# vicpc00/td-vc-gan

Measured on AMD Instinct MI355X. Metric: audio-seconds/sec (G+D train step, stage-1), higher is better.
Workload: dtype f32 (fp32 storage and accumulation everywhere; FiLM cond_var.2 forward and weight-grad as split-bf16 x6 products -- three exact bf16 pieces per operand, six piece products on the bf16 MFMA, fp32 accumulate: fp32-level accuracy; every other kernel exact-fp32 MFMA)

## Files before the change

td-vc-gan_amd/csrc/conv_api.hip:

```cpp
#include "../../include/tdvc.h"
#include "launch.h"
#include "conv_lean.h"
#include "conv_small_group.h"
#include "api_util.h"

using namespace tdvc;

static inline bool al16(const void* p) { return (((uintptr_t)p) & 15) == 0; }
static inline bool ok_bs(const void* p, long bs) { return !p || (bs < (1L << 31)); }
static inline bool vec_ptr(const void* p, long bs) { return !p || (al16(p) && (bs & 3) == 0); }
static inline float scale_or_1(float s) { return s == 0.f ? 1.f : s; }

static int lean_xfk(const tdvc_xform& x, float* slope, float* scale, const float** aux, long* aux_bs) {
  *scale = scale_or_1(x.scale); *aux = x.aux; *aux_bs = x.aux_bs; *slope = x.slope;
  switch (x.kind) {
    case TDVC_XF_NONE: *slope = 1.f; *aux = nullptr; return LXF_ACT;
    case TDVC_XF_LRELU: *aux = nullptr; return (x.slope >= 0.f && x.slope <= 1.f) ? LXF_ACT : -1;
    case TDVC_XF_FILM_LRELU: return (x.slope >= 0.f && x.slope <= 1.f) ? LXF_FILM : -1;
    case TDVC_XF_MASK_LRELU: return LXF_MASK_LRELU;
    case TDVC_XF_MASK_TANH: return LXF_MASK_TANH;
    default: return -1;
  }
}

namespace tdvc { int g_force_generic = 0; }
extern "C" void tdvc_set_force_generic(int on) { g_force_generic = on; }

static Xf to_xf(const tdvc_xform& x) {
  Xf r; r.kind = x.kind; r.slope = x.slope; r.scale = scale_or_1(x.scale);
  r.aux = x.aux; r.aux_bs = x.aux_bs; return r;
}

static int check_desc(const tdvc_conv_desc* d) {
  if (!d) return tdvc_fail(TDVC_EINVAL, "null desc");
  if (d->B <= 0 || d->Cin <= 0 || d->Cout <= 0 || d->Tin <= 0 || d->Tout <= 0 || d->K <= 0 || d->stride <= 0 ||
      d->dilation <= 0 || d->groups <= 0 || d->pad < 0)
    return tdvc_fail(TDVC_EINVAL, "conv desc: non-positive dimension");
  if (d->Cin % d->groups || d->Cout % d->groups) return tdvc_fail(TDVC_EINVAL, "conv desc: channels not divisible by groups");
  if (d->stride > 1 && d->dilation != 1) return tdvc_fail(TDVC_EUNSUPPORTED, "strided conv with dilation");
  if (d->reflect && (d->stride != 1 || d->kind != TDVC_CONV)) return tdvc_fail(TDVC_EUNSUPPORTED, "reflect padding needs stride 1 conv");
  if (d->reflect && d->pad >= d->Tin) return tdvc_fail(TDVC_EINVAL, "reflect padding must be smaller than the input length");
  if (d->w_cin < 0 || d->w_cin_off < 0) return tdvc_fail(TDVC_EINVAL, "conv desc: negative weight channel window");
  if (d->w_cin > 0) {
    if (d->groups != 1 || d->kind != TDVC_CONV) return tdvc_fail(TDVC_EUNSUPPORTED, "weight channel window needs a plain conv with groups == 1");
    if (d->w_cin_off + d->Cin > d->w_cin) return tdvc_fail(TDVC_EINVAL, "conv desc: weight channel window out of range");
  }
  if (d->kind == TDVC_CONV) {
    long expect = ((long)d->Tin + 2L * d->pad - (long)d->dilation * (d->K - 1) - 1) / d->stride + 1;
    if (expect != d->Tout) return tdvc_fail(TDVC_EINVAL, "conv desc: Tout does not match conv arithmetic");
  } else if (d->kind == TDVC_CONV_TRANSPOSE) {
    if (d->stride < 2) return tdvc_fail(TDVC_EUNSUPPORTED, "transposed conv needs stride >= 2");
    long expect = ((long)d->Tin - 1) * d->stride - 2L * d->pad + (d->K - 1) + 1;
    if (d->Tout > expect + d->stride - 1 || d->Tout < expect) return tdvc_fail(TDVC_EINVAL, "conv desc: Tout does not match transposed conv arithmetic");
  } else return tdvc_fail(TDVC_EINVAL, "conv desc: unknown kind");
  return TDVC_OK;
}

static inline int ceil_div(int a, int b) { return (a + b - 1) / b; }

enum { TRY_NEXT = 1 };
static int launch_rc(hipError_t e, bool may_decline = false) {
  if (e == hipSuccess) return TDVC_OK;
  if (may_decline && e == hipErrorNotSupported) return TRY_NEXT;
  return tdvc_fail(TDVC_ELAUNCH, hipGetErrorString(e));
}

template <class P>
static void set_reduced(P& p, int mode, int R, int C, int T, const tdvc_conv_desc* d) {
  const int s = d->stride;
  p.mode = mode; p.R = R; p.Cred = C; p.N = T; p.J = ceil_div(d->K, s); p.d = 1;
  if (mode == MODE_DIRECT) p.d = d->dilation;
  else if (mode == MODE_DOWN) p.Cred = C * s;
  else { p.R = R * s; p.N = (T - 1 + d->pad) / s + 1; }
}

static bool small_group_ok(const tdvc_conv_desc* d) {
  return !g_force_generic && g_knob[2] == 0 && d->kind == TDVC_CONV && d->groups >= 16 && d->Cin == 4 * d->groups && d->Cout == 4 * d->groups &&
         d->dilation == 1 && !d->reflect && d->w_cin == 0 && d->stride >= 2 && d->stride <= 8 && d->K <= 48;
}
static void small_group_base(const tdvc_conv_desc* d, SmallGroupP& q) {
  q.B = d->B; q.G = d->groups; q.Tin = d->Tin; q.Tout = d->Tout; q.K = d->K; q.s = d->stride; q.pad = d->pad;
  q.in_scale = 1.f; q.out_scale = 1.f; q.dy_scale = 1.f;
}

static bool use_mfma(const GemmConvP& p) {
  if (g_force_generic) return false;
  if (p.R <= 2 && p.x.Cg == 1 && p.Cy_g <= 2) return false;
  return (long)p.Cred * p.J >= 7;
}

template <int MODE>
static int run_gemm(GemmConvP& p, int B, hipStream_t st) {
  return launch_rc(use_mfma(p) ? launch_conv_gemm<MODE>(p, B, st) : launch_conv_scalar<MODE>(p, B, st));
}

static int dispatch_gemm(GemmConvP& p, int B, hipStream_t st) {
  switch (p.mode) {
    case MODE_DIRECT: return run_gemm<MODE_DIRECT>(p, B, st);
    case MODE_DOWN: return run_gemm<MODE_DOWN>(p, B, st);
    default: return run_gemm<MODE_UP>(p, B, st);
  }
}

enum { CV_SMALL_GROUP, CV_LEAN, CV_GENERIC };

static bool lean_shape_ok(const tdvc_conv_desc* d) {
  return !g_force_generic && d->kind == TDVC_CONV && d->stride == 1 && d->groups == 1 && d->Tin == d->Tout && ((d->Tin & 3) == 0 || d->Tin <= 80);
}

static bool lean_fill(const tdvc_conv_desc* d, const tdvc_xform& xf, const long (&bs)[7], LeanP& q, int* xfk) {
  long aux_bs;
  *xfk = lean_xfk(xf, &q.slope, &q.in_scale, &q.aux, &aux_bs);
  const struct { const void* p; long bs; int* q_bs; } opnds[] = {{q.x, bs[0], &q.x_bs}, {q.y, bs[1], &q.y_bs}, {q.res, bs[2], &q.res_bs}, {q.add, bs[3], &q.add_bs},
      {q.mx, bs[4], &q.mx_bs}, {q.gb, bs[5], &q.gb_bs}, {q.dgb, bs[6], &q.dgb_bs}, {q.aux, aux_bs, &q.aux_bs}};
  bool ok = *xfk >= 0 && (q.Cw & 3) == 0 && al16(q.w), vec = (d->Tin & 3) == 0;
  for (const auto& o : opnds) { ok = ok && ok_bs(o.p, o.bs); vec = vec && vec_ptr(o.p, o.bs); *o.q_bs = (int)o.bs; }
  q.T = d->Tin; q.K = d->K; q.d = d->dilation; q.vec = vec ? 1 : 0;
  return ok && (vec || d->Tin <= 80);
}

static int fwd_route(const tdvc_conv_desc* d, const tdvc_conv_fwd_args* a, int from, LeanP& q, int* xfk) {
  if (from <= CV_SMALL_GROUP && small_group_ok(d) && a->x_xf.kind <= TDVC_XF_LRELU && !a->res && !a->add && !a->bias3) return CV_SMALL_GROUP;
  if (from <= CV_LEAN && lean_shape_ok(d) && (d->Cin & 3) == 0) {
    q.x = a->x; q.y = a->y; q.bias = a->bias; q.bias3 = a->bias3; q.res = a->res; q.add = a->add;
    q.w = a->w + (long)d->w_cin_off * d->K; q.Cw = (d->w_cin > 0 ? d->w_cin : d->Cin) * d->K;
    q.Cin = d->Cin; q.Cout = d->Cout; q.pad = d->pad; q.reflect = d->reflect;
    q.post = a->post_act; q.out_scale = scale_or_1(a->out_scale); q.add_scale = 1.f; q.m_slope = a->post_slope;
    q.sbits = a->sign_bits; q.sb_bs = (int)a->sign_bits_bs;
    if (lean_fill(d, a->x_xf, {a->x_bs, a->y_bs, a->res_bs, a->add_bs, 0, 0, 0}, q, xfk)) return CV_LEAN;
  }
  return CV_GENERIC;
}

extern "C" int tdvc_conv_fwd(const tdvc_conv_desc* d, const tdvc_conv_fwd_args* a, void* stream) {
  if (int rc = check_desc(d)) return rc;
  if (!a || !a->x || !a->w || !a->y) return tdvc_fail(TDVC_EINVAL, "conv_fwd: null pointer");
  hipStream_t st = (hipStream_t)stream;
  LeanP q = {};
  int xfk = 0, route = CV_SMALL_GROUP;
  while ((route = fwd_route(d, a, route, q, &xfk)) != CV_GENERIC) {
    hipError_t e;
    if (route == CV_SMALL_GROUP) {
      SmallGroupP g = {};
      small_group_base(d, g);
      g.x = a->x; g.x_bs = a->x_bs; g.w = a->w; g.bias = a->bias; g.y = a->y; g.y_bs = a->y_bs;
      g.act_in = a->x_xf.kind == TDVC_XF_LRELU; g.slope_in = a->x_xf.slope; g.in_scale = scale_or_1(a->x_xf.scale);
      g.post = a->post_act; g.post_slope = a->post_slope; g.out_scale = scale_or_1(a->out_scale);
      e = launch_small_group_fwd(g, st);
    } else e = launch_conv_lean(q, d->B, xfk, EPI_FWD, st);
    const int rc = launch_rc(e, true);
    if (rc != TRY_NEXT) return rc;
    ++route;
  }
  if (a->sign_bits) return tdvc_fail(TDVC_EUNSUPPORTED, "conv_fwd: sign_bits needs a stride-1 conv with Tout % 32 == 0, Tout > 80 and 16-byte aligned operands");
  const int Cin_g = d->Cin / d->groups, Cout_g = d->Cout / d->groups;
  GemmConvP p = {};
  p.x.p = a->x; p.x.bs = a->x_bs; p.x.T = d->Tin; p.x.Cg = Cin_g; p.x.xf = to_xf(a->x_xf);
  p.w = a->w; p.K = d->K; p.s = d->stride; p.pad = d->pad; p.groups = d->groups;
  p.y = a->y; p.y_bs = a->y_bs; p.Ty = d->Tout; p.Cy_g = Cout_g;
  p.epi = EPI_FWD; p.bias = a->bias; p.bias3 = a->bias3; p.res = a->res; p.res_bs = a->res_bs;
  p.post = a->post_act; p.post_slope = a->post_slope; p.out_scale = scale_or_1(a->out_scale);
  p.add = a->add; p.add_bs = a->add_bs; p.add_scale = 1.f;
  p.w_sg = (long)Cout_g * Cin_g * d->K;
  if (d->kind == TDVC_CONV) {
    p.w_sm = (long)Cin_g * d->K; p.w_sc = d->K;
    if (d->w_cin > 0) { p.w_sm = (long)d->w_cin * d->K; p.w += (long)d->w_cin_off * d->K; }
    set_reduced(p, d->stride == 1 ? MODE_DIRECT : MODE_DOWN, Cout_g, Cin_g, d->Tout, d);
    p.reflect = d->reflect;
  } else {
    p.w_sm = d->K; p.w_sc = (long)Cout_g * d->K;
    set_reduced(p, MODE_UP, Cout_g, Cin_g, d->Tout, d);
  }
  return dispatch_gemm(p, d->B, st);
}

static int dgrad_route(const tdvc_conv_desc* d, const tdvc_conv_dgrad_args* a, int from, LeanP& q, int* xfk) {
  if (from <= CV_SMALL_GROUP && small_group_ok(d) && a->epilogue == TDVC_DG_PLAIN && !a->add &&
      (a->dy_xf.kind == TDVC_XF_NONE || (a->dy_xf.kind == TDVC_XF_MASK_LRELU && a->dy_xf.aux))) return CV_SMALL_GROUP;
  if (from <= CV_LEAN && a->wt && lean_shape_ok(d) && (d->Cout & 3) == 0 && (d->K - 1) * d->dilation - d->pad >= 0) {
    q.x = a->dy; q.y = a->dx; q.add = a->add; q.mx = a->x_in; q.gb = a->gb; q.dgb = a->dgb;
    q.Cw = d->Cout * d->K; q.w = a->wt + (long)d->w_cin_off * q.Cw;
    q.Cin = d->Cout; q.Cout = d->Cin; q.pad = (d->K - 1) * d->dilation - d->pad; q.flip = 1; q.mirror = d->reflect ? d->pad : 0;
    q.out_scale = 1.f; q.add_scale = a->add_scale; q.m_slope = a->slope;
    if (a->epilogue == TDVC_DG_MASK_LRELU && a->x_sign_bits) { q.mbits = a->x_sign_bits; q.mb_bs = (int)a->x_sign_bits_bs; }
    if (lean_fill(d, a->dy_xf, {a->dy_bs, a->dx_bs, 0, a->add_bs, a->x_in_bs, a->gb_bs, a->dgb_bs}, q, xfk)) return CV_LEAN;
  }
  return CV_GENERIC;
}

extern "C" int tdvc_conv_dgrad(const tdvc_conv_desc* d, const tdvc_conv_dgrad_args* a, void* stream) {
  if (int rc = check_desc(d)) return rc;
  if (!a || !a->dy || !a->w || !a->dx) return tdvc_fail(TDVC_EINVAL, "conv_dgrad: null pointer");
  if (a->epilogue < TDVC_DG_PLAIN || a->epilogue > TDVC_DG_FILM) return tdvc_fail(TDVC_EINVAL, "conv_dgrad: unknown epilogue");
  const int epi = a->epilogue == TDVC_DG_PLAIN ? EPI_PLAIN : (a->epilogue == TDVC_DG_MASK_LRELU ? EPI_MASK : EPI_FILM);
  if (epi == EPI_MASK && !a->x_in && !a->x_sign_bits) return tdvc_fail(TDVC_EINVAL, "conv_dgrad: mask epilogue needs x_in");
  if (epi == EPI_FILM && (!a->x_in || !a->gb || !a->dgb)) return tdvc_fail(TDVC_EINVAL, "conv_dgrad: FiLM epilogue needs x_in, gb, dgb");
  hipStream_t st = (hipStream_t)stream;
  LeanP q = {};
  int xfk = 0, route = CV_SMALL_GROUP;
  while ((route = dgrad_route(d, a, route, q, &xfk)) != CV_GENERIC) {
    hipError_t e;
    if (route == CV_SMALL_GROUP) {
      SmallGroupP g = {};
      small_group_base(d, g);
      g.dy = a->dy; g.dy_bs = a->dy_bs; g.w = a->w; g.y = a->dx; g.y_bs = a->dx_bs;
      g.dy_scale = scale_or_1(a->dy_xf.scale);
      if (a->dy_xf.kind == TDVC_XF_MASK_LRELU) { g.mask = a->dy_xf.aux; g.mask_bs = a->dy_xf.aux_bs; g.m_slope = a->dy_xf.slope; }
      e = launch_small_group_dgrad(g, st);
    } else {
      e = launch_conv_lean(q, d->B, xfk, epi, st);
      if (e == hipErrorNotSupported && q.mbits && a->x_in) {
        q.mbits = nullptr;
        e = launch_conv_lean(q, d->B, xfk, epi, st);
      }
    }
    const int rc = launch_rc(e, true);
    if (rc != TRY_NEXT) return rc;
    ++route;
  }
  if (epi == EPI_MASK && !a->x_in)
    return tdvc_fail(TDVC_EUNSUPPORTED, "conv_dgrad: x_sign_bits without x_in needs a stride-1 conv with Tin % 32 == 0, Tin > 80 and 16-byte aligned operands");
  const int Cin_g = d->Cin / d->groups, Cout_g = d->Cout / d->groups;
  GemmConvP p = {};
  p.x.p = a->dy; p.x.bs = a->dy_bs; p.x.T = d->Tout; p.x.Cg = Cout_g; p.x.xf = to_xf(a->dy_xf);
  p.w = a->w; p.K = d->K; p.s = d->stride; p.pad = d->pad; p.groups = d->groups;
  p.y = a->dx; p.y_bs = a->dx_bs; p.Ty = d->Tin; p.Cy_g = Cin_g;
  p.add = a->add; p.add_bs = a->add_bs; p.add_scale = a->add_scale;
  p.w_sg = (long)Cout_g * Cin_g * d->K;
  p.epi = epi;
  if (epi != EPI_PLAIN) { p.mx = a->x_in; p.mx_bs = a->x_in_bs; p.m_slope = a->slope; }
  if (epi == EPI_FILM) { p.gb = a->gb; p.gb_bs = a->gb_bs; p.dgb = a->dgb; p.dgb_bs = a->dgb_bs; }
  if (d->kind == TDVC_CONV) {
    p.w_sm = d->K; p.w_sc = (long)Cin_g * d->K;
    if (d->w_cin > 0) { p.w_sc = (long)d->w_cin * d->K; p.w += (long)d->w_cin_off * d->K; }
    set_reduced(p, d->stride == 1 ? MODE_DIRECT : MODE_UP, Cin_g, Cout_g, d->Tin, d);
    if (d->stride == 1) {
      p.tap_flip = 1; p.pad = (d->K - 1) * d->dilation - d->pad;
      if (p.pad < 0) return tdvc_fail(TDVC_EUNSUPPORTED, "conv_dgrad: padding larger than the receptive field");
      p.mirror_pad = d->reflect ? d->pad : 0;
    }
  } else {
    p.w_sm = (long)Cout_g * d->K; p.w_sc = d->K;
    set_reduced(p, MODE_DOWN, Cin_g, Cout_g, d->Tin, d);
  }
  return dispatch_gemm(p, d->B, st);
}

static void fill_wgrad(const tdvc_conv_desc* d, const tdvc_conv_wgrad_args* a, WgradP& p) {
  const int Cin_g = d->Cin / d->groups, Cout_g = d->Cout / d->groups;
  p.groups = d->groups; p.K = d->K; p.s = d->stride; p.pad = d->pad;
  p.w_sg = (long)Cout_g * Cin_g * d->K; p.w_sc = d->K;
  if (d->kind == TDVC_CONV) {
    if (a) { p.a.p = a->dy; p.a.bs = a->dy_bs; p.a.xf = to_xf(a->dy_xf); p.x.p = a->x; p.x.bs = a->x_bs; p.x.xf = to_xf(a->x_xf); }
    p.a.T = d->Tout; p.a.Cg = Cout_g; p.x.T = d->Tin; p.x.Cg = Cin_g;
    p.w_sm = (long)Cin_g * d->K;
    set_reduced(p, d->stride == 1 ? MODE_DIRECT : MODE_DOWN, Cout_g, Cin_g, d->Tout, d);
    p.reflect = d->reflect;
  } else {
    if (a) { p.a.p = a->x; p.a.bs = a->x_bs; p.a.xf = to_xf(a->x_xf); p.x.p = a->dy; p.x.bs = a->dy_bs; p.x.xf = to_xf(a->dy_xf); }
    p.a.T = d->Tin; p.a.Cg = Cin_g; p.x.T = d->Tout; p.x.Cg = Cout_g;
    p.w_sm = (long)Cout_g * d->K;
    set_reduced(p, MODE_DOWN, Cin_g, Cout_g, d->Tin, d);
  }
}

static bool wgrad_use_mfma(const WgradP& p) {
  if (g_force_generic) return false;
  if (p.R <= 2 && p.x.Cg == 1) return false;
  if (!wgrad_mfma_supported(p.J)) return false;
  return true;
}

static bool wgrad_lean_ok(const tdvc_conv_desc* d) {
  const bool wide = d->Cout >= 32 && d->Cin >= 32;
  return !g_force_generic && d->kind == TDVC_CONV && d->stride == 1 && d->groups == 1 && d->Tin == d->Tout &&
         (d->Tout > 128 || wide) && wgrad_lean_supported(d->Cout, d->Cin, d->K, d->dilation);
}

static bool wgrad_x6_desc_ok(const tdvc_conv_desc* d) {
  return wgrad_lean_ok(d) && d->w_cin == 0 && wgrad_x6_ok(d->Cout, d->Cin, d->Tout, d->K, d->dilation, d->pad, d->reflect);
}

enum { WG_SMALL_GROUP, WG_X6, WG_LEAN, WG_MFMA, WG_SCALAR };
struct WgPlan {
  int route;
  int nslab; long sstride;
  bool bias;
  int bpb;
  size_t bytes;
};

static WgPlan wgrad_plan(const tdvc_conv_desc* d, const tdvc_conv_wgrad_args* a, WgradP& p, int from) {
  const long wsize = (long)d->groups * p.w_sg;
  WgPlan pl = {};
  auto slabs = [&](int route, int nslab, bool bias) {
    pl.route = route; pl.nslab = nslab; pl.bias = bias; pl.sstride = wsize + (bias ? d->Cout : 0);
    pl.bytes = (size_t)nslab * (size_t)pl.sstride * sizeof(float);
    return pl;
  };
  if (from <= WG_SMALL_GROUP && small_group_ok(d) &&
      (!a || (a->x_xf.kind <= TDVC_XF_LRELU && (a->dy_xf.kind == TDVC_XF_NONE || (a->dy_xf.kind == TDVC_XF_MASK_LRELU && a->dy_xf.aux))))) {
    pl.route = WG_SMALL_GROUP; pl.bias = true; pl.bytes = small_group_wgrad_workspace(d->B, d->groups, d->K);
    return pl;
  }
  if (from <= WG_X6 && wgrad_x6_desc_ok(d) &&
      (!a || (a->x_xf.kind <= TDVC_XF_LRELU && a->dy_xf.kind == TDVC_XF_NONE && scale_or_1(a->x_xf.scale) == 1.f && scale_or_1(a->dy_xf.scale) == 1.f &&
              (a->x_xf.kind == TDVC_XF_NONE || (a->x_xf.slope > 0.f && a->x_xf.slope <= 1.f)) &&
              al16(a->x) && al16(a->dy) && (a->x_bs & 3) == 0 && (a->dy_bs & 3) == 0))) {
    int nt, tpb, nslab;
    wgrad_x6_plan(d->Cout, d->Tout, d->B, &nt, &tpb, &nslab);
    return slabs(WG_X6, nslab, true);
  }
  if (from <= WG_LEAN && wgrad_lean_ok(d)) return slabs(WG_LEAN, wgrad_lean_nslab(d->Cout, d->Cin, d->Tout, d->K, d->B), true);
  if (from <= WG_MFMA && wgrad_use_mfma(p)) {
    const int nslab = wgrad_geometry(p, d->B, &pl.bpb);
    return slabs(WG_MFMA, nslab, false);
  }
  pl.route = WG_SCALAR;
  return pl;
}

extern "C" size_t tdvc_conv_wgrad_workspace(const tdvc_conv_desc* d) {
  if (check_desc(d)) return 0;
  WgradP p = {};
  fill_wgrad(d, nullptr, p);
  size_t need = 0;
  for (int from = WG_SMALL_GROUP; from <= WG_LEAN; ) {
    const WgPlan pl = wgrad_plan(d, nullptr, p, from);
    if (pl.bytes > need) need = pl.bytes;
    from = pl.route + 1;
  }
  return need;
}

extern "C" int tdvc_conv_wgrad(const tdvc_conv_desc* d, const tdvc_conv_wgrad_args* a, void* stream) {
  if (int rc = check_desc(d)) return rc;
  if (!a || !a->x || !a->dy) return tdvc_fail(TDVC_EINVAL, "conv_wgrad: null pointer");
  hipStream_t st = (hipStream_t)stream;
  WgradP p = {};
  fill_wgrad(d, a, p);
  const long wsize = (long)d->groups * p.w_sg;
  float* dw = (a->dw && d->w_cin > 0) ? a->dw + (long)d->w_cin_off * d->K : a->dw;
  const long dw_rs = d->w_cin > 0 ? (long)d->w_cin * d->K : p.w_sm;
  bool bias_done = false;
  for (int from = WG_SMALL_GROUP; a->dw; ) {
    const WgPlan pl = wgrad_plan(d, a, p, from);
    if (pl.route != WG_SMALL_GROUP && pl.bytes && (!a->workspace || a->workspace_bytes < pl.bytes))
      return tdvc_fail(TDVC_EWORKSPACE, "conv_wgrad: workspace too small");
    hipError_t e;
    if (pl.route == WG_SMALL_GROUP) {
      SmallGroupP q = {};
      small_group_base(d, q);
      q.x = a->x; q.x_bs = a->x_bs; q.dy = a->dy; q.dy_bs = a->dy_bs;
      q.act_in = a->x_xf.kind == TDVC_XF_LRELU; q.slope_in = a->x_xf.slope; q.in_scale = scale_or_1(a->x_xf.scale);
      q.dy_scale = scale_or_1(a->dy_xf.scale);
      if (a->dy_xf.kind == TDVC_XF_MASK_LRELU) { q.mask = a->dy_xf.aux; q.mask_bs = a->dy_xf.aux_bs; q.m_slope = a->dy_xf.slope; }
      e = launch_small_group_wgrad(q, a->dw, a->dbias, a->workspace, a->workspace_bytes, st);
    } else if (pl.route == WG_X6 || pl.route == WG_LEAN) {
      WgLeanP q = {};
      q.a = p.a; q.x = p.x; q.R = d->Cout; q.Cin = d->Cin; q.N = d->Tout; q.pad = d->pad; q.K = d->K; q.reflect = d->reflect;
      q.slab = (float*)a->workspace; q.slab_stride = pl.sstride; q.bias_off = a->dbias ? wsize : -1;
      auto okp = [](const Opnd& o) { return al16(o.p) && (o.bs & 3) == 0 && (o.T & 3) == 0 && (!o.xf.aux || (al16(o.xf.aux) && (o.xf.aux_bs & 3) == 0)); };
      q.vec = (okp(q.a) && okp(q.x)) ? 1 : 0;
      e = pl.route == WG_X6 ? launch_conv_wgrad_x6(q, d->B, st) : launch_conv_wgrad_lean(q, d->B, d->K, d->dilation, st);
    } else if (pl.route == WG_MFMA) {
      p.slab = (float*)a->workspace; p.slab_stride = wsize;
      e = p.mode == MODE_DIRECT ? launch_conv_wgrad<MODE_DIRECT>(p, d->B, pl.bpb, st) : launch_conv_wgrad<MODE_DOWN>(p, d->B, pl.bpb, st);
    } else {
      p.w_sm = dw_rs;
      e = p.mode == MODE_DIRECT ? launch_conv_wgrad_scalar<MODE_DIRECT>(p, d->B, wsize, dw, st)
                                : launch_conv_wgrad_scalar<MODE_DOWN>(p, d->B, wsize, dw, st);
    }
    int rc = launch_rc(e, pl.route == WG_SMALL_GROUP || pl.route == WG_LEAN);
    if (rc == TRY_NEXT) { from = pl.route + 1; continue; }
    if (rc == TDVC_OK && pl.nslab)
      rc = launch_rc(launch_slab_reduce((const float*)a->workspace, pl.nslab, pl.sstride, pl.bias && a->dbias ? pl.sstride : wsize, dw, (int)p.w_sm, dw_rs,
                                        st, wsize, pl.bias ? a->dbias : nullptr));
    if (rc) return rc;
    bias_done = pl.bias;
    break;
  }
  if (a->dbias && !bias_done) {
    Opnd dy; dy.p = a->dy; dy.bs = a->dy_bs; dy.T = d->Tout; dy.Cg = d->Cout / d->groups; dy.xf = to_xf(a->dy_xf);
    return launch_rc(launch_bias_grad(dy, d->Tout, d->Cout, d->B, a->dbias, st));
  }
  return TDVC_OK;
}


extern "C" int tdvc_film_cond_fwd(const tdvc_film_cond_args* a, void* stream) {
  if (!a || !a->exc || !a->w0 || !a->k3 || !a->w2 || !a->gb) return tdvc_fail(TDVC_EINVAL, "film_cond_fwd: null pointer");
  if (a->B <= 0 || a->T < 4 || a->n_cond <= a->n_var || a->n_var <= 0 || a->C2 <= 0) return tdvc_fail(TDVC_EINVAL, "film_cond_fwd: bad shape");
  LeanP q = {};
  q.x = a->exc; q.x_bs = (int)a->exc_bs; q.w = a->w2; q.bias = a->b2; q.y = a->gb; q.y_bs = (int)a->gb_bs;
  q.T = a->T; q.Cin = a->n_cond; q.Cout = a->C2; q.Cw = a->n_cond * 3; q.K = 3; q.d = 1; q.pad = 1;
  q.cw = a->w0 + (long)(a->n_cond - a->n_var) * 3; q.cw_stride = a->n_cond * 3; q.Cv = a->n_var;
  q.k3 = a->k3; q.cv0 = a->cv0; q.cv0_bs = (int)a->cv0_bs;
  q.slope = a->slope; q.in_scale = 1.f; q.out_scale = 1.f; q.add_scale = 1.f; q.m_slope = a->slope; q.post = TDVC_POST_NONE;
  q.vec = ((a->T & 3) == 0 && vec_ptr(a->gb, a->gb_bs) && vec_ptr(a->cv0, a->cv0_bs) && al16(a->w2) && ((a->n_cond * 3) & 3) == 0) ? 1 : 0;
  hipError_t e = launch_conv_lean_cond(q, a->B, (hipStream_t)stream);
  if (e == hipErrorNotSupported) return tdvc_fail(TDVC_EUNSUPPORTED, "film_cond_fwd: shape outside the fused kernel's contract");
  return e == hipSuccess ? TDVC_OK : tdvc_fail(TDVC_ELAUNCH, hipGetErrorString(e));
}

extern "C" void tdvc_fold_defer(int on) { tdvc::fold_set_defer(on); }
extern "C" void tdvc_fold_reset(void* stream) { tdvc::fold_reset((hipStream_t)stream); }
extern "C" int tdvc_fold_flush(void* stream) { return launch_rc(tdvc::fold_flush((hipStream_t)stream)); }
```

td-vc-gan_amd/csrc/conv_small_group.h:

```cpp
#pragma once
#include <hip/hip_runtime.h>

namespace tdvc {

struct SmallGroupP {
  const float* x; long x_bs;
  const float* w;
  const float* bias;
  const float* mask; long mask_bs;
  float* y; long y_bs;
  const float* dy; long dy_bs;
  float* slab; long slab_stride;
  int B, G, Tin, Tout, K, s, pad, J;
  int act_in; float slope_in;
  int post; float post_slope; float in_scale, out_scale, dy_scale; float m_slope;
  int CS;
  int nsplit;
};

hipError_t launch_small_group_fwd(SmallGroupP p, hipStream_t st);
hipError_t launch_small_group_dgrad(SmallGroupP p, hipStream_t st);
hipError_t launch_small_group_wgrad(SmallGroupP p, float* dw, float* dbias, void* workspace, size_t workspace_bytes, hipStream_t st);
size_t small_group_wgrad_workspace(int B, int G, int K);

}
```

td-vc-gan_amd/csrc/conv_small_group.hip:

```cpp
#include "launch.h"
#include "conv_small_group.h"

namespace tdvc {

typedef float f32x4 __attribute__((ext_vector_type(4)));

__device__ __forceinline__ float bload(srd_t rs, int elem, bool ok) {
  return __builtin_bit_cast(float, __builtin_amdgcn_raw_buffer_load_b32(rs, ok ? elem * 4 : 0x7f000000, 0, 0));
}

template <int S>
__global__ __launch_bounds__(256) void small_group_fwd_kernel(const SmallGroupP p) {
  extern __shared__ __attribute__((aligned(16))) float smem[];
  const int tid = threadIdx.x, lane = tid & 63, wave = tid >> 6;
  const int g = blockIdx.x * 4 + wave, b = blockIdx.y, t0 = blockIdx.z * 64;
  const int xsz = 4 * S * p.CS, wsz = 16 * p.K;
  float* xs = smem + wave * (xsz + wsz);
  float* ws = xs + xsz;
  const bool live = g < p.G;
  if (live) {
    const float* wg = p.w + (long)g * 16 * p.K;
    float wv[12];
    const srd_t wrs = make_srd(wg, 16 * p.K * 4);
#pragma unroll
    for (int i = 0; i < 12; ++i) { const int e = lane + i * 64; wv[i] = bload(wrs, e, e < 16 * p.K); }
    const int q0 = t0 * S - p.pad, span = 63 * S + p.K;
    const float inv_s = 1.0f / (float)S;
    const srd_t xrs = make_srd(p.x + (long)b * p.x_bs + (long)(g * 4) * p.Tin, 4 * p.Tin * 4);
    for (int e0 = 0; e0 < span; e0 += 5 * 64) {
      float xv[4][5];
#pragma unroll
      for (int ci = 0; ci < 4; ++ci)
#pragma unroll
        for (int i = 0; i < 5; ++i) {
          const int e = e0 + lane + i * 64, q = q0 + e;
          xv[ci][i] = bload(xrs, ci * p.Tin + q, e < span && q >= 0 && q < p.Tin);
        }
#pragma unroll
      for (int ci = 0; ci < 4; ++ci)
#pragma unroll
        for (int i = 0; i < 5; ++i) {
          const int e = e0 + lane + i * 64;
          if (e < span) {
            float v = xv[ci][i];
            if (p.act_in) v = fmaxf(v, v * p.slope_in);
            const int col = (int)(((float)e + 0.5f) * inv_s);
            xs[(ci * S + (e - col * S)) * p.CS + col] = v * p.in_scale;
          }
        }
    }
#pragma unroll
    for (int i = 0; i < 12; ++i) {
      const int e = lane + i * 64;
      if (e < 16 * p.K) { const int co = e / (4 * p.K), r = e - co * 4 * p.K; ws[r * 4 + co] = wv[i]; }
    }
  }
  __syncthreads();
  if (!live) return;
  f32x4 acc = {0.f, 0.f, 0.f, 0.f};
  for (int ci = 0; ci < 4; ++ci) {
    const float* xc = xs + ci * S * p.CS + lane;
    const f32x4* wc = reinterpret_cast<const f32x4*>(ws) + ci * p.K;
    for (int j = 0; j < p.J; ++j) {
      float xv4[S]; f32x4 w4[S];
#pragma unroll
      for (int phi = 0; phi < S; ++phi) {
        const bool ok = j * S + phi < p.K;
        xv4[phi] = ok ? xc[phi * p.CS + j] : 0.f;
        w4[phi] = ok ? wc[j * S + phi] : (f32x4){0.f, 0.f, 0.f, 0.f};
      }
#pragma unroll
      for (int phi = 0; phi < S; ++phi) acc += w4[phi] * xv4[phi];
    }
  }
  const int t = t0 + lane;
  if (t >= p.Tout) return;
#pragma unroll
  for (int co = 0; co < 4; ++co) {
    const int ch = g * 4 + co;
    float v = acc[co] + (p.bias ? p.bias[ch] : 0.f);
    if (p.post == POST_LRELU) v = lrelu_f(v, p.post_slope);
    else if (p.post == POST_TANH) v = tanhf(v);
    p.y[(long)b * p.y_bs + (long)ch * p.Tout + t] = v * p.out_scale;
  }
}

template <int S>
__global__ __launch_bounds__(256) void small_group_dgrad_kernel(const SmallGroupP p) {
  extern __shared__ __attribute__((aligned(16))) float smem[];
  const int tid = threadIdx.x, lane = tid & 63, wave = tid >> 6;
  const int g = blockIdx.x * 4 + wave, b = blockIdx.y, m0 = blockIdx.z * 64;
  const int DS = 64 + p.J;
  const int dsz = 4 * DS, wsz = 16 * p.J * S;
  float* ds = smem + wave * (dsz + wsz);
  float* ws = ds + dsz;
  const bool live = g < p.G;
  if (live) {
    const float* wg = p.w + (long)g * 16 * p.K;
    float wv[12];
    const srd_t wrs = make_srd(wg, 16 * p.K * 4);
    const srd_t drs = make_srd(p.dy + (long)b * p.dy_bs + (long)(g * 4) * p.Tout, 4 * p.Tout * 4);
    const srd_t mrs = make_srd(p.mask ? p.mask + (long)b * p.mask_bs + (long)(g * 4) * p.Tout : p.dy, p.mask ? 4 * p.Tout * 4 : 0);
#pragma unroll
    for (int i = 0; i < 12; ++i) {
      const int e = lane + i * 64;
      const int ci = e & 3; int rest = e >> 2;
      const int r = rest % S; rest /= S;
      const int j = rest % p.J, co = rest / p.J;
      const int k = r + j * S;
      wv[i] = bload(wrs, (co * 4 + ci) * p.K + k, e < wsz && k < p.K);
    }
    float dv[4][2], mv[4][2];
#pragma unroll
    for (int co = 0; co < 4; ++co)
#pragma unroll
      for (int i = 0; i < 2; ++i) {
        const int e = lane + i * 64, t = m0 - p.J + 1 + e;
        const bool ok = e < DS && t >= 0 && t < p.Tout;
        dv[co][i] = bload(drs, co * p.Tout + t, ok);
        mv[co][i] = bload(mrs, co * p.Tout + t, ok);
      }
#pragma unroll
    for (int i = 0; i < 12; ++i) { const int e = lane + i * 64; if (e < wsz) ws[e] = wv[i]; }
#pragma unroll
    for (int co = 0; co < 4; ++co)
#pragma unroll
      for (int i = 0; i < 2; ++i) {
        const int e = lane + i * 64;
        if (e < DS) { const float v = dv[co][i] * p.dy_scale; ds[co * DS + e] = (!p.mask || mv[co][i] > 0.f) ? v : v * p.m_slope; }
      }
  }
  __syncthreads();
  if (!live) return;
  f32x4 acc[S];
#pragma unroll
  for (int r = 0; r < S; ++r) acc[r] = (f32x4){0.f, 0.f, 0.f, 0.f};
  for (int co = 0; co < 4; ++co) {
    const float* dc = ds + co * DS + lane + p.J - 1;
    const f32x4* wc = reinterpret_cast<const f32x4*>(ws) + co * p.J * S;
#pragma unroll 2
    for (int j = 0; j < p.J; ++j) {
      const float dv = dc[-j];
#pragma unroll
      for (int r = 0; r < S; ++r) acc[r] += wc[j * S + r] * dv;
    }
  }
  const int m = m0 + lane;
  const int u0 = m * S - p.pad;
  if (u0 >= p.Tin || u0 + S <= 0) return;
  float* dxb = p.y + (long)b * p.y_bs + (long)(g * 4) * p.Tin;
  const bool vec = S == 4 && u0 >= 0 && u0 + 3 < p.Tin && ((u0 | p.Tin) & 3) == 0 && (p.y_bs & 3) == 0 && (((uintptr_t)p.y) & 15) == 0;
#pragma unroll
  for (int ci = 0; ci < 4; ++ci) {
    if (vec) {
      if (S == 4) *reinterpret_cast<f32x4*>(dxb + (long)ci * p.Tin + u0) = (f32x4){acc[0][ci], acc[1 % S][ci], acc[2 % S][ci], acc[3 % S][ci]} * p.out_scale;
    } else {
#pragma unroll
      for (int r = 0; r < S; ++r)
        if (u0 + r >= 0 && u0 + r < p.Tin) dxb[(long)ci * p.Tin + u0 + r] = acc[r][ci] * p.out_scale;
    }
  }
}

__global__ __launch_bounds__(256) void small_group_wgrad_kernel(const SmallGroupP p) {
  extern __shared__ __attribute__((aligned(16))) float smem[];
  const int tid = threadIdx.x;
  const int g = blockIdx.x, split = blockIdx.y;
  const int XW = p.Tin + 2 * p.pad + p.s;
  float* xs = smem;
  float* ds = xs + 4 * XW;
  const int nel = 16 * p.K;
  const int e_ci = tid / p.K, e_k = tid - e_ci * p.K;
  const bool e_live = tid < 4 * p.K;
  f32x4 acc = {0.f, 0.f, 0.f, 0.f};
  float bacc = 0.f;
  int xo[6]; bool xk[6];
#pragma unroll
  for (int u = 0; u < 6; ++u) {
    const int i = tid + u * 256;
    const int ci = i / XW, q = i - ci * XW - p.pad;
    xk[u] = i < 4 * XW && q >= 0 && q < p.Tin;
    xo[u] = ci * p.Tin + q;
  }
  const bool dk = tid < 4 * p.Tout;
  float xv[6], dv, mv;
  auto issue = [&](int b) {
    const srd_t xrs = make_srd(p.x + (long)b * p.x_bs + (long)(g * 4) * p.Tin, 4 * p.Tin * 4);
    const srd_t drs = make_srd(p.dy + (long)b * p.dy_bs + (long)(g * 4) * p.Tout, 4 * p.Tout * 4);
    const srd_t mrs = make_srd(p.mask ? p.mask + (long)b * p.mask_bs + (long)(g * 4) * p.Tout : p.dy, p.mask ? 4 * p.Tout * 4 : 0);
#pragma unroll
    for (int u = 0; u < 6; ++u) xv[u] = bload(xrs, xo[u], xk[u]);
    dv = bload(drs, tid, dk);
    mv = bload(mrs, tid, dk);
  };
  issue(split);
  for (int b = split; b < p.B; b += p.nsplit) {
    __syncthreads();
#pragma unroll
    for (int u = 0; u < 6; ++u) {
      const int i = tid + u * 256;
      if (i < 4 * XW) { float v = xv[u]; if (p.act_in) v = fmaxf(v, v * p.slope_in); xs[i] = v * p.in_scale; }
    }
    if (dk) {
      const float v = dv * p.dy_scale;
      const int co = tid / p.Tout, t = tid - co * p.Tout;
      ds[t * 4 + co] = (!p.mask || mv > 0.f) ? v : v * p.m_slope;
    }
    __syncthreads();
    if (b + p.nsplit < p.B) issue(b + p.nsplit);
    if (e_live) {
      const f32x4* dr = reinterpret_cast<const f32x4*>(ds);
      const float* xr = xs + e_ci * XW + e_k;
      f32x4 s0 = {0.f, 0.f, 0.f, 0.f}, s1 = {0.f, 0.f, 0.f, 0.f};
      int t = 0;
      for (; t + 1 < p.Tout; t += 2) { s0 += dr[t] * xr[t * p.s]; s1 += dr[t + 1] * xr[(t + 1) * p.s]; }
      if (t < p.Tout) s0 += dr[t] * xr[t * p.s];
      acc += s0 + s1;
    }
    if (tid >= 252) {
      float sb = 0.f;
      for (int t = 0; t < p.Tout; ++t) sb += ds[t * 4 + (tid - 252)];
      bacc += sb;
    }
  }
  float* slab = p.slab + (long)split * p.slab_stride;
  if (e_live) {
#pragma unroll
    for (int co = 0; co < 4; ++co) slab[(long)g * nel + (co * 4 + e_ci) * p.K + e_k] = acc[co];
  }
  if (tid >= 252) slab[(long)p.G * nel + g * 4 + (tid - 252)] = bacc;
}

static inline int sg_cs(int s, int K) { return ((64 + (K + s - 1) / s + 1 + 15) / 16) * 16; }

hipError_t launch_small_group_fwd(SmallGroupP p, hipStream_t st) {
  p.J = (p.K + p.s - 1) / p.s;
  p.CS = sg_cs(p.s, p.K);
  const size_t lds = (size_t)4 * (4 * p.s * p.CS + 16 * p.K) * sizeof(float);
  if (lds > 64 * 1024 || 16 * p.K > 768) return hipErrorNotSupported;
  const dim3 grid((p.G + 3) / 4, p.B, (p.Tout + 63) / 64);
  if (p.s == 2) { TDVC_TRACE(small_group_fwd_kernel<2>); hipLaunchKernelGGL(small_group_fwd_kernel<2>, grid, dim3(256), lds, st, p); }
  else if (p.s == 4) { TDVC_TRACE(small_group_fwd_kernel<4>); hipLaunchKernelGGL(small_group_fwd_kernel<4>, grid, dim3(256), lds, st, p); }
  else if (p.s == 8) { TDVC_TRACE(small_group_fwd_kernel<8>); hipLaunchKernelGGL(small_group_fwd_kernel<8>, grid, dim3(256), lds, st, p); }
  else return hipErrorNotSupported;
  return hipGetLastError();
}

hipError_t launch_small_group_dgrad(SmallGroupP p, hipStream_t st) {
  p.J = (p.K + p.s - 1) / p.s;
  if (p.s > 8 || 16 * p.J * p.s > 768 || p.J > 64) return hipErrorNotSupported;
  const size_t lds = (size_t)4 * (4 * (64 + p.J) + 16 * p.J * p.s) * sizeof(float);
  if (lds > 64 * 1024) return hipErrorNotSupported;
  const int M = (p.Tin - 1 + p.pad) / p.s + 1;
  const dim3 grid((p.G + 3) / 4, p.B, (M + 63) / 64);
  if (p.s == 2) { TDVC_TRACE(small_group_dgrad_kernel<2>); hipLaunchKernelGGL(small_group_dgrad_kernel<2>, grid, dim3(256), lds, st, p); }
  else if (p.s == 4) { TDVC_TRACE(small_group_dgrad_kernel<4>); hipLaunchKernelGGL(small_group_dgrad_kernel<4>, grid, dim3(256), lds, st, p); }
  else if (p.s == 8) { TDVC_TRACE(small_group_dgrad_kernel<8>); hipLaunchKernelGGL(small_group_dgrad_kernel<8>, grid, dim3(256), lds, st, p); }
  else return hipErrorNotSupported;
  return hipGetLastError();
}

size_t small_group_wgrad_workspace(int B, int G, int K) {
  const int nsplit = B >= 8 ? 4 : 1;
  return (size_t)nsplit * ((size_t)G * 16 * K + (size_t)G * 4) * sizeof(float);
}

hipError_t launch_small_group_wgrad(SmallGroupP p, float* dw, float* dbias, void* workspace, size_t workspace_bytes, hipStream_t st) {
  if (4 * p.K > 252 || 4 * (p.Tin + 2 * p.pad + p.s) > 6 * 256 || 4 * p.Tout > 256) return hipErrorNotSupported;
  p.nsplit = p.B >= 8 ? 4 : 1;
  const long nW = (long)p.G * 16 * p.K, n = nW + (long)p.G * 4;
  if (workspace_bytes < (size_t)p.nsplit * n * sizeof(float) || !workspace) return hipErrorNotSupported;
  const size_t lds = (size_t)(4 * (p.Tin + 2 * p.pad + p.s) + 4 * p.Tout) * sizeof(float);
  if (lds > 64 * 1024) return hipErrorNotSupported;
  p.slab = (float*)workspace; p.slab_stride = n;
  TDVC_TRACE(small_group_wgrad_kernel);
  hipLaunchKernelGGL(small_group_wgrad_kernel, dim3(p.G, p.nsplit), dim3(256), lds, st, p);
  hipError_t e = hipGetLastError();
  if (e != hipSuccess) return e;
  return launch_slab_reduce(p.slab, p.nsplit, n, dbias ? n : nW, dw, (int)nW, nW, st, nW, dbias);
}

}
```

Before: 301.1.

## Add MFMA kernels for grouped stride-4 convs with 4-in/16-out channels per group

Adds a dedicated route for grouped strided convolutions with 4 input and 16 output channels per group (stride 4, K up to 44), covering both forward and data-gradient. Each single-wave block stages its group's weights in LDS, keeps them in registers, prefetches the next time tile, and accumulates with fp32 16x16x4 MFMA. Tiles per block are sized so the grid roughly fills the device. These shapes previously fell to the generic GEMM path; the new kernels add code, and their one-wave blocks may limit latency hiding.

```diff
diff --git a/td-vc-gan_amd/csrc/conv_api.hip b/td-vc-gan_amd/csrc/conv_api.hip
--- a/td-vc-gan_amd/csrc/conv_api.hip
+++ b/td-vc-gan_amd/csrc/conv_api.hip
@@ -78,6 +78,10 @@
   return !g_force_generic && g_knob[2] == 0 && d->kind == TDVC_CONV && d->groups >= 16 && d->Cin == 4 * d->groups && d->Cout == 4 * d->groups &&
          d->dilation == 1 && !d->reflect && d->w_cin == 0 && d->stride >= 2 && d->stride <= 8 && d->K <= 48;
 }
+static bool group16_ok(const tdvc_conv_desc* d) {
+  return !g_force_generic && g_knob[2] == 0 && d->kind == TDVC_CONV && d->groups >= 4 && d->Cin == 4 * d->groups && d->Cout == 16 * d->groups &&
+         d->stride == 4 && d->K <= 44 && (d->pad & 3) == 0 && d->dilation == 1 && !d->reflect && d->w_cin == 0;
+}
 static void small_group_base(const tdvc_conv_desc* d, SmallGroupP& q) {
   q.B = d->B; q.G = d->groups; q.Tin = d->Tin; q.Tout = d->Tout; q.K = d->K; q.s = d->stride; q.pad = d->pad;
   q.in_scale = 1.f; q.out_scale = 1.f; q.dy_scale = 1.f;
@@ -102,7 +106,7 @@
   }
 }
 
-enum { CV_SMALL_GROUP, CV_LEAN, CV_GENERIC };
+enum { CV_SMALL_GROUP, CV_GROUP16, CV_LEAN, CV_GENERIC };
 
 static bool lean_shape_ok(const tdvc_conv_desc* d) {
   return !g_force_generic && d->kind == TDVC_CONV && d->stride == 1 && d->groups == 1 && d->Tin == d->Tout && ((d->Tin & 3) == 0 || d->Tin <= 80);
@@ -121,6 +125,7 @@
 
 static int fwd_route(const tdvc_conv_desc* d, const tdvc_conv_fwd_args* a, int from, LeanP& q, int* xfk) {
   if (from <= CV_SMALL_GROUP && small_group_ok(d) && a->x_xf.kind <= TDVC_XF_LRELU && !a->res && !a->add && !a->bias3) return CV_SMALL_GROUP;
+  if (from <= CV_GROUP16 && group16_ok(d) && a->x_xf.kind <= TDVC_XF_LRELU && !a->res && !a->add && !a->bias3) return CV_GROUP16;
   if (from <= CV_LEAN && lean_shape_ok(d) && (d->Cin & 3) == 0) {
     q.x = a->x; q.y = a->y; q.bias = a->bias; q.bias3 = a->bias3; q.res = a->res; q.add = a->add;
     q.w = a->w + (long)d->w_cin_off * d->K; q.Cw = (d->w_cin > 0 ? d->w_cin : d->Cin) * d->K;
@@ -140,13 +145,13 @@
   int xfk = 0, route = CV_SMALL_GROUP;
   while ((route = fwd_route(d, a, route, q, &xfk)) != CV_GENERIC) {
     hipError_t e;
-    if (route == CV_SMALL_GROUP) {
+    if (route == CV_SMALL_GROUP || route == CV_GROUP16) {
       SmallGroupP g = {};
       small_group_base(d, g);
       g.x = a->x; g.x_bs = a->x_bs; g.w = a->w; g.bias = a->bias; g.y = a->y; g.y_bs = a->y_bs;
       g.act_in = a->x_xf.kind == TDVC_XF_LRELU; g.slope_in = a->x_xf.slope; g.in_scale = scale_or_1(a->x_xf.scale);
       g.post = a->post_act; g.post_slope = a->post_slope; g.out_scale = scale_or_1(a->out_scale);
-      e = launch_small_group_fwd(g, st);
+      e = route == CV_GROUP16 ? launch_group16_fwd(g, st) : launch_small_group_fwd(g, st);
     } else e = launch_conv_lean(q, d->B, xfk, EPI_FWD, st);
     const int rc = launch_rc(e, true);
     if (rc != TRY_NEXT) return rc;
@@ -177,6 +182,8 @@
 static int dgrad_route(const tdvc_conv_desc* d, const tdvc_conv_dgrad_args* a, int from, LeanP& q, int* xfk) {
   if (from <= CV_SMALL_GROUP && small_group_ok(d) && a->epilogue == TDVC_DG_PLAIN && !a->add &&
       (a->dy_xf.kind == TDVC_XF_NONE || (a->dy_xf.kind == TDVC_XF_MASK_LRELU && a->dy_xf.aux))) return CV_SMALL_GROUP;
+  if (from <= CV_GROUP16 && group16_ok(d) && a->epilogue == TDVC_DG_PLAIN && !a->add &&
+      (a->dy_xf.kind == TDVC_XF_NONE || (a->dy_xf.kind == TDVC_XF_MASK_LRELU && a->dy_xf.aux))) return CV_GROUP16;
   if (from <= CV_LEAN && a->wt && lean_shape_ok(d) && (d->Cout & 3) == 0 && (d->K - 1) * d->dilation - d->pad >= 0) {
     q.x = a->dy; q.y = a->dx; q.add = a->add; q.mx = a->x_in; q.gb = a->gb; q.dgb = a->dgb;
     q.Cw = d->Cout * d->K; q.w = a->wt + (long)d->w_cin_off * q.Cw;
@@ -200,13 +207,13 @@
   int xfk = 0, route = CV_SMALL_GROUP;
   while ((route = dgrad_route(d, a, route, q, &xfk)) != CV_GENERIC) {
     hipError_t e;
-    if (route == CV_SMALL_GROUP) {
+    if (route == CV_SMALL_GROUP || route == CV_GROUP16) {
       SmallGroupP g = {};
       small_group_base(d, g);
       g.dy = a->dy; g.dy_bs = a->dy_bs; g.w = a->w; g.y = a->dx; g.y_bs = a->dx_bs;
       g.dy_scale = scale_or_1(a->dy_xf.scale);
       if (a->dy_xf.kind == TDVC_XF_MASK_LRELU) { g.mask = a->dy_xf.aux; g.mask_bs = a->dy_xf.aux_bs; g.m_slope = a->dy_xf.slope; }
-      e = launch_small_group_dgrad(g, st);
+      e = route == CV_GROUP16 ? launch_group16_dgrad(g, st) : launch_small_group_dgrad(g, st);
     } else {
       e = launch_conv_lean(q, d->B, xfk, epi, st);
       if (e == hipErrorNotSupported && q.mbits && a->x_in) {
diff --git a/td-vc-gan_amd/csrc/conv_small_group.h b/td-vc-gan_amd/csrc/conv_small_group.h
--- a/td-vc-gan_amd/csrc/conv_small_group.h
+++ b/td-vc-gan_amd/csrc/conv_small_group.h
@@ -16,10 +16,13 @@
   int post; float post_slope; float in_scale, out_scale, dy_scale; float m_slope;
   int CS;
   int nsplit;
+  int tpr;
 };
 
 hipError_t launch_small_group_fwd(SmallGroupP p, hipStream_t st);
 hipError_t launch_small_group_dgrad(SmallGroupP p, hipStream_t st);
+hipError_t launch_group16_fwd(SmallGroupP p, hipStream_t st);
+hipError_t launch_group16_dgrad(SmallGroupP p, hipStream_t st);
 hipError_t launch_small_group_wgrad(SmallGroupP p, float* dw, float* dbias, void* workspace, size_t workspace_bytes, hipStream_t st);
 size_t small_group_wgrad_workspace(int B, int G, int K);
 
diff --git a/td-vc-gan_amd/csrc/conv_small_group.hip b/td-vc-gan_amd/csrc/conv_small_group.hip
--- a/td-vc-gan_amd/csrc/conv_small_group.hip
+++ b/td-vc-gan_amd/csrc/conv_small_group.hip
@@ -4,6 +4,7 @@
 namespace tdvc {
 
 typedef float f32x4 __attribute__((ext_vector_type(4)));
+typedef float f32x2 __attribute__((ext_vector_type(2)));
 
 __device__ __forceinline__ float bload(srd_t rs, int elem, bool ok) {
   return __builtin_bit_cast(float, __builtin_amdgcn_raw_buffer_load_b32(rs, ok ? elem * 4 : 0x7f000000, 0, 0));
@@ -231,6 +232,220 @@
   if (tid >= 252) slab[(long)p.G * nel + g * 4 + (tid - 252)] = bacc;
 }
 
+constexpr int G16_KMAX = 44, G16_JMAX = 11;
+constexpr int G16_NCOL = 64 + G16_JMAX - 1;
+constexpr int G16_XCS = 80, G16_DCS = 80;
+constexpr int G16_WAVES = 256 * 14;
+static inline int g16_tpr(int B, int G, int ntile) {
+  long tpr = ((long)B * G * ntile + G16_WAVES - 1) / G16_WAVES;
+  tpr = tpr < 1 ? 1 : (tpr > ntile ? ntile : tpr);
+  const long nruns = (ntile + tpr - 1) / tpr;
+  return (int)((ntile + nruns - 1) / nruns);
+}
+
+__device__ __forceinline__ void g16_wave_sync() {
+  __builtin_amdgcn_fence(__ATOMIC_RELEASE, "wavefront"); __builtin_amdgcn_wave_barrier(); __builtin_amdgcn_fence(__ATOMIC_ACQUIRE, "wavefront");
+}
+
+__device__ __forceinline__ void g16_stage_weights(const float* wg, int K, float* ws, int lane) {
+  const srd_t wrs = make_srd(wg, 64 * K * 4);
+  float wv[G16_KMAX];
+#pragma unroll
+  for (int i = 0; i < G16_KMAX; ++i) wv[i] = bload(wrs, lane + i * 64, true);
+#pragma unroll
+  for (int i = 0; i < G16_KMAX; ++i) ws[lane + i * 64] = wv[i];
+  g16_wave_sync();
+}
+
+template <int JT>
+__global__ __launch_bounds__(64) void group16_fwd_kernel(const SmallGroupP p) {
+  extern __shared__ __attribute__((aligned(16))) float smem[];
+  const int lane = threadIdx.x, ln = lane & 15, kq = lane >> 4;
+  const int g = blockIdx.x, b = blockIdx.y;
+  const int ntile = (p.Tout + 63) >> 6;
+  const int tile0 = blockIdx.z * p.tpr, tile1 = min(tile0 + p.tpr, ntile);
+  const srd_t xrs = make_srd(p.x + (long)b * p.x_bs + (long)(g * 4) * p.Tin, 4 * p.Tin * 4);
+  const int lw = (lane & 3) * G16_XCS + (lane >> 2);
+  float pre[20];
+  auto issue = [&](int tile) {
+    const int qb = tile * 256 - p.pad + lane;
+#pragma unroll
+    for (int ci = 0; ci < 4; ++ci)
+#pragma unroll
+      for (int i = 0; i < 5; ++i) {
+        const int q = qb + 64 * i;
+        pre[ci * 5 + i] = bload(xrs, ci * p.Tin + q, (unsigned)q < (unsigned)p.Tin && (i < 4 || lane < 4 * G16_NCOL - 256));
+      }
+  };
+  issue(tile0);
+  constexpr int NJ = JT ? JT : G16_JMAX;
+  float w[NJ * 4];
+  g16_stage_weights(p.w + (long)g * 64 * p.K, p.K, smem, lane);
+#pragma unroll
+  for (int j = 0; j < NJ; ++j)
+#pragma unroll
+    for (int ci = 0; ci < 4; ++ci) {
+      const int k = 4 * j + kq;
+      w[j * 4 + ci] = k < p.K ? smem[(ln * 4 + ci) * p.K + k] : 0.f;
+    }
+  g16_wave_sync();
+  const int ch = g * 16 + ln;
+  const float bias = p.bias ? p.bias[ch] : 0.f;
+  float* yr = p.y + (long)b * p.y_bs + (long)ch * p.Tout;
+  const bool vec4 = (p.Tout & 3) == 0 && (p.y_bs & 3) == 0 && (((uintptr_t)p.y) & 15) == 0;
+  const bool vec2 = (p.Tout & 1) == 0 && (p.y_bs & 1) == 0 && (((uintptr_t)p.y) & 7) == 0;
+  for (int tile = tile0; tile < tile1; ++tile) {
+#pragma unroll
+    for (int ci = 0; ci < 4; ++ci)
+#pragma unroll
+      for (int i = 0; i < 5; ++i)
+        if (i < 4 || lane < 4 * G16_NCOL - 256) {
+          float v = pre[ci * 5 + i];
+          if (p.act_in) v = fmaxf(v, v * p.slope_in);
+          smem[lw + ci * 4 * G16_XCS + 16 * i] = v * p.in_scale;
+        }
+    g16_wave_sync();
+    if (tile + 1 < tile1) issue(tile + 1);
+    f32x4 acc[4];
+#pragma unroll
+    for (int n = 0; n < 4; ++n) acc[n] = (f32x4){0.f, 0.f, 0.f, 0.f};
+    const float* xb = smem + kq * G16_XCS + ln;
+    float xv[3][4];
+#pragma unroll
+    for (int n = 0; n < 4; ++n) { xv[0][n] = xb[n * 16]; xv[1][n] = xb[4 * G16_XCS + n * 16]; }
+#pragma unroll
+    for (int j = 0; j < NJ; ++j) {
+      if (JT || j < p.J) {
+#pragma unroll
+        for (int s = 4 * j; s < 4 * j + 4; ++s) {
+          if (s + 2 < NJ * 4) {
+            const float* xk = xb + ((s + 2) & 3) * 4 * G16_XCS + ((s + 2) >> 2);
+#pragma unroll
+            for (int n = 0; n < 4; ++n) xv[(s + 2) % 3][n] = xk[n * 16];
+          }
+#pragma unroll
+          for (int n = 0; n < 4; ++n) acc[n] = __builtin_amdgcn_mfma_f32_16x16x4f32(xv[s % 3][n], w[s], acc[n], 0, 0, 0);
+          __builtin_amdgcn_sched_barrier(0);
+        }
+      }
+    }
+    g16_wave_sync();
+#pragma unroll
+    for (int n = 0; n < 4; ++n) {
+      const int t = tile * 64 + n * 16 + kq * 4;
+      if (t >= p.Tout) continue;
+      f32x4 v = acc[n] + bias;
+#pragma unroll
+      for (int q = 0; q < 4; ++q) v[q] = p.post == POST_LRELU ? lrelu_f(v[q], p.post_slope) : v[q];
+      v *= p.out_scale;
+      if (vec4) *reinterpret_cast<f32x4*>(yr + t) = v;
+      else if (vec2 && t + 3 < p.Tout) {
+        *reinterpret_cast<f32x2*>(yr + t) = (f32x2){v[0], v[1]};
+        *reinterpret_cast<f32x2*>(yr + t + 2) = (f32x2){v[2], v[3]};
+      } else {
+#pragma unroll
+        for (int q = 0; q < 4; ++q)
+          if (t + q < p.Tout) yr[t + q] = v[q];
+      }
+    }
+  }
+}
+
+template <int JT>
+__global__ __launch_bounds__(64) void group16_dgrad_kernel(const SmallGroupP p) {
+  extern __shared__ __attribute__((aligned(16))) float smem[];
+  const int lane = threadIdx.x, ln = lane & 15, kq = lane >> 4;
+  const int g = blockIdx.x, b = blockIdx.y;
+  const int M = (p.Tin - 1 + p.pad) / 4 + 1, ntile = (M + 63) >> 6;
+  const int tile0 = blockIdx.z * p.tpr, tile1 = min(tile0 + p.tpr, ntile);
+  const srd_t drs = make_srd(p.dy + (long)b * p.dy_bs + (long)(g * 16) * p.Tout, 16 * p.Tout * 4);
+  const srd_t mrs = make_srd(p.mask ? p.mask + (long)b * p.mask_bs + (long)(g * 16) * p.Tout : p.dy, 16 * p.Tout * 4);
+  const int rsel = lane >> 5, c = lane & 31;
+  const int lw = rsel * G16_DCS + c;
+  float pre[24], prm[24];
+  auto issue = [&](int tile) {
+    const int tb = tile * 64 - (G16_JMAX - 1) + c;
+#pragma unroll
+    for (int pr = 0; pr < 8; ++pr)
+#pragma unroll
+      for (int i = 0; i < 3; ++i) {
+        const int t = tb + 32 * i, off = (2 * pr + rsel) * p.Tout + t;
+        const bool ok = (unsigned)t < (unsigned)p.Tout && (i < 2 || c < G16_NCOL - 64);
+        pre[pr * 3 + i] = bload(drs, off, ok);
+        prm[pr * 3 + i] = p.mask ? bload(mrs, off, ok) : 1.f;
+      }
+  };
+  issue(tile0);
+  constexpr int NJ = JT ? JT : G16_JMAX;
+  float w[NJ * 4];
+  g16_stage_weights(p.w + (long)g * 64 * p.K, p.K, smem, lane);
+  {
+    const int ci = ln >> 2, r = ln & 3;
+#pragma unroll
+    for (int j = 0; j < NJ; ++j)
+#pragma unroll
+      for (int cq = 0; cq < 4; ++cq) {
+        const int k = r + 4 * j;
+        w[j * 4 + cq] = k < p.K ? smem[((cq * 4 + kq) * 4 + ci) * p.K + k] : 0.f;
+      }
+  }
+  g16_wave_sync();
+  float* dxr = p.y + (long)b * p.y_bs + (long)(g * 4 + kq) * p.Tin;
+  const bool vec4 = (p.Tin & 3) == 0 && (p.y_bs & 3) == 0 && (((uintptr_t)p.y) & 15) == 0;
+  const bool vec2 = (p.Tin & 1) == 0 && (p.y_bs & 1) == 0 && (((uintptr_t)p.y) & 7) == 0;
+  for (int tile = tile0; tile < tile1; ++tile) {
+#pragma unroll
+    for (int pr = 0; pr < 8; ++pr)
+#pragma unroll
+      for (int i = 0; i < 3; ++i)
+        if (i < 2 || c < G16_NCOL - 64) {
+          const float v = pre[pr * 3 + i];
+          smem[lw + 2 * pr * G16_DCS + 32 * i] = (prm[pr * 3 + i] > 0.f ? v : v * p.m_slope) * p.dy_scale;
+        }
+    g16_wave_sync();
+    if (tile + 1 < tile1) issue(tile + 1);
+    f32x4 acc[4];
+#pragma unroll
+    for (int n = 0; n < 4; ++n) acc[n] = (f32x4){0.f, 0.f, 0.f, 0.f};
+    const float* db = smem + kq * G16_DCS + ln + (G16_JMAX - 1);
+    auto dptr = [&](int s) { return db + (s & 3) * 4 * G16_DCS - (NJ - 1 - (s >> 2)); };
+    float dv[3][4];
+#pragma unroll
+    for (int s = 0; s < NJ * 4; ++s) {
+      const int j = NJ - 1 - (s >> 2);
+      if (JT || j < p.J) {
+        if ((s & 3) == 0 && (s == 0 || (!JT && j == p.J - 1))) {
+#pragma unroll
+          for (int n = 0; n < 4; ++n) { dv[s % 3][n] = dptr(s)[n * 16]; dv[(s + 1) % 3][n] = dptr(s + 1)[n * 16]; }
+        }
+        if (s + 2 < NJ * 4) {
+#pragma unroll
+          for (int n = 0; n < 4; ++n) dv[(s + 2) % 3][n] = dptr(s + 2)[n * 16];
+        }
+#pragma unroll
+        for (int n = 0; n < 4; ++n) acc[n] = __builtin_amdgcn_mfma_f32_16x16x4f32(w[j * 4 + (s & 3)], dv[s % 3][n], acc[n], 0, 0, 0);
+        __builtin_amdgcn_sched_barrier(0);
+      }
+    }
+    g16_wave_sync();
+#pragma unroll
+    for (int n = 0; n < 4; ++n) {
+      const int u0 = (tile * 64 + n * 16 + ln) * 4 - p.pad;
+      if (u0 >= p.Tin || u0 < 0) continue;
+      const f32x4 v = acc[n] * p.out_scale;
+      if (vec4) *reinterpret_cast<f32x4*>(dxr + u0) = v;
+      else if (vec2 && u0 + 3 < p.Tin) {
+        *reinterpret_cast<f32x2*>(dxr + u0) = (f32x2){v[0], v[1]};
+        *reinterpret_cast<f32x2*>(dxr + u0 + 2) = (f32x2){v[2], v[3]};
+      } else {
+#pragma unroll
+        for (int r = 0; r < 4; ++r)
+          if (u0 + r < p.Tin) dxr[u0 + r] = v[r];
+      }
+    }
+  }
+}
+
 static inline int sg_cs(int s, int K) { return ((64 + (K + s - 1) / s + 1 + 15) / 16) * 16; }
 
 hipError_t launch_small_group_fwd(SmallGroupP p, hipStream_t st) {
@@ -257,6 +472,37 @@
   else if (p.s == 4) { TDVC_TRACE(small_group_dgrad_kernel<4>); hipLaunchKernelGGL(small_group_dgrad_kernel<4>, grid, dim3(256), lds, st, p); }
   else if (p.s == 8) { TDVC_TRACE(small_group_dgrad_kernel<8>); hipLaunchKernelGGL(small_group_dgrad_kernel<8>, grid, dim3(256), lds, st, p); }
   else return hipErrorNotSupported;
+  return hipGetLastError();
+}
+
+static bool group16_launchable(const SmallGroupP& p) {
+  return p.s == 4 && p.K >= 1 && p.K <= G16_KMAX && p.pad >= 0 && (p.pad & 3) == 0 && p.B <= 65535 && p.G >= 1;
+}
+static constexpr size_t G16_LDS = (size_t)64 * G16_KMAX * sizeof(float);
+
+hipError_t launch_group16_fwd(SmallGroupP p, hipStream_t st) {
+  if (!group16_launchable(p) || p.post == POST_TANH) return hipErrorNotSupported;
+  p.J = (p.K + 3) / 4;
+  const int ntile = (p.Tout + 63) / 64;
+  p.tpr = g16_tpr(p.B, p.G, ntile);
+  const dim3 grid(p.G, p.B, (ntile + p.tpr - 1) / p.tpr);
+  if (grid.z > 65535) return hipErrorNotSupported;
+  const size_t lds = G16_LDS;
+  if (p.J == G16_JMAX) { TDVC_TRACE(group16_fwd_kernel<G16_JMAX>); hipLaunchKernelGGL(group16_fwd_kernel<G16_JMAX>, grid, dim3(64), lds, st, p); }
+  else { TDVC_TRACE(group16_fwd_kernel<0>); hipLaunchKernelGGL(group16_fwd_kernel<0>, grid, dim3(64), lds, st, p); }
+  return hipGetLastError();
+}
+
+hipError_t launch_group16_dgrad(SmallGroupP p, hipStream_t st) {
+  if (!group16_launchable(p)) return hipErrorNotSupported;
+  p.J = (p.K + 3) / 4;
+  const int M = (p.Tin - 1 + p.pad) / 4 + 1, ntile = (M + 63) / 64;
+  p.tpr = g16_tpr(p.B, p.G, ntile);
+  const dim3 grid(p.G, p.B, (ntile + p.tpr - 1) / p.tpr);
+  if (grid.z > 65535) return hipErrorNotSupported;
+  const size_t lds = G16_LDS;
+  if (p.J == G16_JMAX) { TDVC_TRACE(group16_dgrad_kernel<G16_JMAX>); hipLaunchKernelGGL(group16_dgrad_kernel<G16_JMAX>, grid, dim3(64), lds, st, p); }
+  else { TDVC_TRACE(group16_dgrad_kernel<0>); hipLaunchKernelGGL(group16_dgrad_kernel<0>, grid, dim3(64), lds, st, p); }
   return hipGetLastError();
 }
 
```

New measurement: 308.0, median of 6. +2.3%, better.
